# Aaron20127/human-3d-reconstruction

Hardware: AMD Instinct MI355X
Metric: images/sec whole-node, DLA-34+SMPL batch-64 512x512; top-k index bit-match (higher is better)
Workload: dtype bf16; 1 GPU; DLA-34+DCNv2 multi_pose + pose/shape heads -> sigmoid/NMS/top-100 decode -> SMPL 6890-vert LBS; 512x512, batch 64 per GPU (BASELINE configs[2]); batch_per_gpu=64, global_batch=64, K=100, smpl_people_per_image=100, parallelism=dp1 (image shards, one all-gather of dets), collective=none (one rank), steps_in_flight=3, hip_graph=False, dcn_margin=auto, images=64 distinct synthetic images (h3d_amd.synth.synth_image_batch, seed 317), weights=synthetic (h3d_amd.synth, seed 0, gain 1.25, offset_scale 0.5)

## Files before the change

human-3d-reconstruction_amd/_lib.py:

```python
import ctypes
import os

_HERE = os.path.dirname(os.path.abspath(__file__))
LIB_PATH = os.path.join(_HERE, "csrc", "libh3d_hip.so")

H3D_F32, H3D_BF16, H3D_F16, H3D_F16X3 = 0, 1, 2, 3
OP_STEM, OP_CONV, OP_DCN, OP_MAXPOOL, OP_UPADD, OP_COPY, OP_HEADS, OP_DCN_V1, OP_DCN_FUSED = 1, 2, 3, 4, 5, 6, 7, 8, 9
OP_CONV_STREAM, OP_DCN_FUSED_F16, OP_DCN_FUSED_STREAM, OP_STEM3, OP_UPDCN_F16 = 10, 11, 12, 13, 14
OP_IM2COL, OP_MAXPOOL3, OP_DEPTH2SPACE = 15, 16, 17
HEADS_MAX = 16
OUT_NHWC, OUT_NCHW_F32, OUT_NHWC_F32, OUT_NHWC_F16 = 0, 1, 2, 3
DCN_INPUT_NHWC, DCN_OUTPUT_NHWC, DCN_F32_MFMA = 1, 2, 4
ABI_VERSION = 4

DCN_AUX_BYTES = 256
DCN_FUSED_BIAS_WMAX, DCN_FUSED_BIAS_AMAX = 32, 34
OPF_DCN_MASK_FINAL, OPF_DCN_RAW_PACK, OPF_DCN_ACT_MAXIMA, TUNE_DCN_ABLATE_MASK = 0x800, 0x100000, 0x200000, 0x1f
OPF_DCN_FUSED_RAW_PACK, OPF_DCN_FUSED_SCALED_INPUT = 0x100000, 0x200000
TUNE_DCN_FUSED_X3_MARGIN2, TUNE_DCN_FUSED_X3_MARGIN6, TUNE_DCN_FUSED_X3_MARGIN4, TUNE_DCN_FUSED_X3_ABLATE_MASK = 0x2000, 0x4000, 0x8000, 0x1f
OPF_DCN_STREAM_NO_SLOTS, OPF_DCN_STREAM_WIDE_MARGIN, OPF_DCN_STREAM_SLOTS512, OPF_DCN_STREAM_F16_INPUT = 0x1000, 0x8000, 0x10000, 0x40000
OPF_DCN_STREAM_STATS, OPF_DCN_STREAM_VARIANT_MASK = 0x20000, 0x58600
TUNE_DCN_STREAM_FORCE_NARROW_WG, TUNE_DCN_STREAM_FORCE_WIDE_WG = 0x200, 0x400
TUNE_DCN_STREAM_F16_DCN5, TUNE_DCN_STREAM_F16_KEEP_DCN3, TUNE_DCN_STREAM_ABLATE_MASK = 0x4000, 0x2000, 0x1f
TUNE_DCN_STREAM_X3_MARGIN2, TUNE_DCN_STREAM_X3_MARGIN3, TUNE_DCN_STREAM_X3_MARGIN4, TUNE_DCN_STREAM_X3_ABLATE_MASK = 0x4000, 0x8000, 0x10000, 0x1f
TUNE_DCN_F16_ONE_WG_PER_CU, TUNE_DCN_F16_ABLATE_MASK = 0x100, 0xff
TUNE_CONV_STREAM_TILE_MASK, TUNE_CONV_STREAM_AUTO, TUNE_CONV_STREAM_ROUND4_RULE, TUNE_CONV_STREAM_ABLATE_MASK = 0xffff, 1, 0x10000000, 0x1f0000
TUNE_CONV_TILE, TUNE_CONV_HALO_TILE, TUNE_CONV_FORCE_GEMM, TUNE_CONV_GEMM_TILE_MASK = 0x1000, 0x2000, 0x4000, 0xf00
TUNE_CONV_X3_TILED, TUNE_CONV_X3_TILE_MASK, TUNE_CONV_X3_CK16, TUNE_CONV_X3_MT2 = 0x1000, 0x1fff, 0x2000, 0x4000
TUNE_UPADD_TAPS_GLOBAL, TUNE_UPADD_TAPS_LDS = 1, 2
TUNE_HEADS_SEPARATE_BIAS, TUNE_HEADS_ABLATE_MASK = 0x200, 0xff


def TUNE_DCN_STREAM_DCN5_XP(xp):
    return xp << 16


def TUNE_DCN_STREAM_DCN5_XP_OF(reserved):
    return (reserved >> 16) & 0xff


def TUNE_CONV_STREAM_TILE(variant, mt, waves):
    return variant << 12 | mt << 8 | waves


def TUNE_CONV_STREAM_ABLATE(bits):
    return bits << 16


def TUNE_CONV_STREAM_ABLATE_OF(reserved):
    return (reserved & TUNE_CONV_STREAM_ABLATE_MASK) >> 16


def TUNE_CONV_1X1_TILE(mt, th):
    return TUNE_CONV_TILE | mt << 4 | th >> 3


def TUNE_CONV_1X1_TILE_MT(reserved):
    return (reserved >> 4) & 15


def TUNE_CONV_1X1_TILE_TH(reserved):
    return (reserved & 15) * 8


def TUNE_CONV_GEMM_TILE(n):
    return n << 8


def TUNE_CONV_X3_TILE(mt, waves, th):
    return TUNE_CONV_X3_TILED | mt << 8 | waves << 4 | th >> 3

c_vp, c_i, c_fp = ctypes.c_void_p, ctypes.c_int, ctypes.c_void_p


class H3dOp(ctypes.Structure):
    _fields_ = [
        ("kind", ctypes.c_int32), ("dtype", ctypes.c_int32),
        ("in_", c_vp), ("in2", c_vp), ("w", c_vp), ("bias", c_vp), ("out", c_vp),
        ("B", ctypes.c_int32), ("H", ctypes.c_int32), ("W", ctypes.c_int32),
        ("Cin", ctypes.c_int32), ("in_cs", ctypes.c_int32), ("in2_cs", ctypes.c_int32),
        ("Ho", ctypes.c_int32), ("Wo", ctypes.c_int32),
        ("Cout", ctypes.c_int32), ("out_cs", ctypes.c_int32),
        ("ksize", ctypes.c_int32), ("stride", ctypes.c_int32), ("relu", ctypes.c_int32),
        ("out_mode", ctypes.c_int32), ("wrows", ctypes.c_int32), ("reserved", ctypes.c_int32),
        ("wexp", ctypes.c_int32), ("wexp2", ctypes.c_int32),
    ]


class _HeadEntry(ctypes.Structure):
    _fields_ = [("w2", c_vp), ("b2", c_vp), ("out", c_vp), ("C", ctypes.c_int32), ("wexp2", ctypes.c_int32)]


class H3dHeadsDesc(ctypes.Structure):
    _fields_ = [("nheads", ctypes.c_int32), ("wexp", ctypes.c_int32), ("head", _HeadEntry * HEADS_MAX)]


HEADS_LISTS_MAX = 4


class H3dHeadsList(ctypes.Structure):
    _fields_ = [("inds", c_vp), ("K", ctypes.c_int32), ("head_mask", ctypes.c_uint32)]


class H3dUpdcnDesc(ctypes.Structure):
    _fields_ = [("skip", c_vp), ("w_up", c_vp), ("w_off", c_vp), ("skip_cs", ctypes.c_int32), ("reserved", ctypes.c_int32)]


TRAIN_BRIGHTNESS, TRAIN_CONTRAST, TRAIN_SATURATION = 0, 1, 2
TRAIN_INPUT_NO_COLOR_AUG = 1


class H3dTrainImage(ctypes.Structure):
    _fields_ = [("minv", ctypes.c_double * 6), ("light", ctypes.c_double * 3), ("offset", ctypes.c_int64),
# ... 164 lines not shown
```

human-3d-reconstruction_amd/csrc/heads.hip:

```cpp
#include "common.h"
#include <string.h>
#include <type_traits>
#include <utility>

constexpr int HEADS_MAX = 16;
constexpr int HC_IN = 64;
constexpr int HC_SLAB = 64;
constexpr int HC_MT2 = 3;
constexpr int HEADS_LISTS_MAX = 4;
#ifndef HEADS_PF_WIDE
#define HEADS_PF_WIDE 0
#endif
#ifndef HEADS_PF
#define HEADS_PF 2
#endif

#ifndef HEADS_SPARSE_NW
#define HEADS_SPARSE_NW 8
#endif
static_assert(HEADS_SPARSE_NW == 4 || HEADS_SPARSE_NW == 8, "sparse heads: 24 wave-instructions per stage in whole numbers per wave, at most 512 threads");

struct HeadsArgs {
    const char *in;
    const char *w1;
    const float *b1;
    const char *w2[HEADS_MAX];
    const float *b2[HEADS_MAX];
    float *out[HEADS_MAX];
    int C[HEADS_MAX];
    int nheads, head_conv;
    int B, H, W, in_cs;
    int tiles_x, tiles_y;
    int dbg;
    int xcd;
    float s1;
    float s2[HEADS_MAX];
    unsigned long long *stamps;
    int nlists;
    const long long *l_inds[HEADS_LISTS_MAX];
    int l_K[HEADS_LISTS_MAX], l_wg0[HEADS_LISTS_MAX], l_nh[HEADS_LISTS_MAX];
    int l_head[HEADS_LISTS_MAX][HEADS_MAX];
};

template <typename T, int TH>
struct HeadsCfg {
    static constexpr int TW = 32;
    static constexpr int ES = sizeof(T);
    static constexpr int NT = TH / 8;
    static constexpr int NW = 8;
    static constexpr int IN_H = TH + 2, IN_W = TW + 2;
    static constexpr int SB = HC_IN * ES + 16;
    static constexpr int RB = IN_W * SB;
    static constexpr int RBW = HC_IN * ES;
    static constexpr int CPR = RBW / 16;
    static constexpr int SWZ_SHIFT = ES == 2 ? 1 : 0;
    static constexpr int TAPS = ES == 2 ? 3 : 1;
    static constexpr int TRS = 9 / TAPS;
    static constexpr int SLOT = TAPS * HC_SLAB * RBW;
    static constexpr int LDS_IN = IN_H * RB;
    static constexpr int LDS_W2 = 32 * HC_MT2 * RBW;
    static constexpr int LDS_BIAS = 1024 + 1024;
    static constexpr int LDS = LDS_IN + 2 * SLOT + LDS_W2 + 2 * LDS_BIAS;
    static constexpr int RPI = 1024 / RBW;
    static constexpr int VPR = HC_IN * ES / 16;
};

template <typename T>
struct HeadsSparseCfg {
    using D = HeadsCfg<T, 16>;
    static_assert(sizeof(T) == 2, "sparse heads: 2-byte plans");
    static constexpr int ES = D::ES, NT = 1, TW = D::TW;
    static constexpr int CW = 2, NW = HEADS_SPARSE_NW;
    static constexpr int NPOS = 32 * CW;
    static constexpr int SB = D::SB, RB = 3 * SB, PB = 3 * RB;
    static constexpr int RBW = D::RBW, CPR = D::CPR, SWZ_SHIFT = D::SWZ_SHIFT, TAPS = D::TAPS, TRS = D::TRS, SLOT = D::SLOT;
    static constexpr int LDS_IN = NPOS * PB;
    static constexpr int LDS_W2 = D::LDS_W2, LDS_BIAS = D::LDS_BIAS;
    static constexpr int LDS = LDS_IN + 2 * SLOT + LDS_W2 + 2 * LDS_BIAS;
    static constexpr int RPI = D::RPI, VPR = D::VPR;
    static_assert(LDS <= 160 * 1024, "LDS of a CU");
};

template <int OFF>
__device__ __forceinline__ void lds_read16_async(u32x4 &dst, uint32_t addr)
{
    static_assert(OFF >= 0 && OFF < 65536, "ds_read offset field");
    asm volatile("ds_read_b128 %0, %1 offset:%2" : "=v"(dst) : "v"(addr), "n"(OFF));
}
template <class F, int... I>
__device__ __forceinline__ void static_for_impl(F &&f, std::integer_sequence<int, I...>) { (f(std::integral_constant<int, I>{}), ...); }
template <int N, class F>
__device__ __forceinline__ void static_for(F &&f) { static_for_impl(f, std::make_integer_sequence<int, N>{}); }

__device__ __forceinline__ void heads_issue_bias(const float *b1, int hc, const float *b2, char *dst, int wv, int l)
{
    if (wv == 0) {
        const auto rs = __builtin_amdgcn_make_buffer_rsrc((void *)b1, 0, hc * 4, 0x00020000);
        __builtin_amdgcn_raw_ptr_buffer_load_lds(rs, (__attribute__((address_space(3))) void *)dst, 16, l * 16, 0, 0, 0);
    } else if (wv == 1) {
        const auto rs = __builtin_amdgcn_make_buffer_rsrc((void *)b2, 0, 96 * 4, 0x00020000);
        __builtin_amdgcn_raw_ptr_buffer_load_lds(rs, (__attribute__((address_space(3))) void *)(dst + 1024), 16, l * 16 < 512 ? l * 16 : 0x7ffffff0, 0, 0, 0);
    }
}

template <typename T, int TH, int NT, int M2, bool BIASC>
__device__ __forceinline__ void gemm2(f32x16 (&acc)[2][NT], f32x16 (&acc2)[M2][NT], const char *s_b1 ,
                                      const char *s_w2, int r, int h, int sw, float s1 = 1.f)
{
    using C = HeadsCfg<T, TH>;
    using E = ET<T>;
    constexpr int ES = sizeof(T);
    typedef short s16x2 __attribute__((ext_vector_type(2)));
#pragma unroll
    for (int m = 0; m < 2; ++m) {
#pragma unroll
        for (int sb = 0; sb < 2; ++sb) {
            typename E::frag fb[NT];
            float bias[8] = {0.f, 0.f, 0.f, 0.f, 0.f, 0.f, 0.f, 0.f};
            if constexpr (!BIASC) {
                const f32x4 b_lo = *reinterpret_cast<const f32x4 *>(s_b1 + (m * 32 + 16 * sb + 4 * h) * 4);
                const f32x4 b_hi = *reinterpret_cast<const f32x4 *>(s_b1 + (m * 32 + 16 * sb + 4 * h + 8) * 4);
#pragma unroll
                for (int j = 0; j < 4; ++j) { bias[j] = b_lo[j]; bias[4 + j] = b_hi[j]; }
// ... 363 lines not shown
                else if ((H3D_DBG(a) & 8) && wv < 4) {  }
                else if (BIASC && tr == 0) stage(std::true_type{}, slot, tr);
                else stage(std::false_type{}, slot, tr);
#ifdef H3D_ABLATE
                t_stage += __builtin_readcyclecounter() - ts0;
#endif
#ifdef H3D_ABLATE
                const unsigned long long tb0 = __builtin_readcyclecounter();
                __builtin_amdgcn_s_waitcnt(0x0f70);
                const unsigned long long tb1 = __builtin_readcyclecounter();
                t_dma += tb1 - tb0;
#endif
                if (!(H3D_DBG(a) & 2))
                __syncthreads();
#ifdef H3D_ABLATE
                t_bar += __builtin_readcyclecounter() - tb1;
#endif
            }
#ifdef H3D_ABLATE
            const unsigned long long tg0 = __builtin_readcyclecounter();
#endif
            if (!(SPARSE && idle))
            gemm2<T, TH, NT, M2H, BIASC>(acc, acc2, s_b + slab * HC_SLAB * 4, s_w2, r, h, sw, a.s1);
#ifdef H3D_ABLATE
            t_g2 += __builtin_readcyclecounter() - tg0;
#endif
            if (C::TRS == 1) __syncthreads();
        }
        const int C_head = a.C[head];
        float *out = a.out[head];
        const size_t cstride = (size_t)a.H * a.W;
        [[maybe_unused]] const float s2 = a.s2[head];
#pragma unroll
        for (int n = 0; n < NT; ++n) {
            const int oy = SPARSE ? sp_y : oy0 + wv * NT + n, ox = SPARSE ? sp_x : ox0 + r, ob = SPARSE ? sp_b : b;
            if (SPARSE ? sp_ok : oy < a.H && ox < a.W) {
                float *op = out + (((size_t)ob * C_head + 4 * h) * a.H + oy) * a.W + ox;
#pragma unroll
                for (int m2 = 0; m2 < M2H; ++m2) {
#pragma unroll
                    for (int g = 0; g < 4; ++g) {
                        const int c = m2 * 32 + 8 * g + 4 * h;
                        float *p = op + (size_t)(m2 * 32 + 8 * g) * cstride;
                        const f32x4 b2v = *reinterpret_cast<const f32x4 *>(s_b + 1024 + c * 4);
#pragma unroll
                        for (int i = 0; i < 4; ++i)
                            if (c + i < C_head) {
                                if constexpr (std::is_same_v<T, x3_t>) p[i * cstride] = fmaf(acc2[m2][n][4 * g + i], s2, b2v[i]);
                                else p[i * cstride] = acc2[m2][n][4 * g + i] + b2v[i];
                            }
                        __builtin_amdgcn_sched_barrier(0);
                    }
                }
            }
        }
        };
    for (int hi = 0; hi < nh; ++hi) {
        const int head = head_at(hi);
        if constexpr (!MIXED) {
            head_body(std::integral_constant<int, M2>{}, hi, head);
        } else {
            const int m2h = __builtin_amdgcn_readfirstlane((a.C[head] + 31) >> 5);
            if (m2h <= 1) head_body(std::integral_constant<int, 1>{}, hi, head);
            else if (M2 < 3 || m2h == 2) head_body(std::integral_constant<int, (M2 < 2 ? 1 : 2)>{}, hi, head);
            else head_body(std::integral_constant<int, M2>{}, hi, head);
        }
    }
#ifdef H3D_ABLATE
    if (a.stamps && blockIdx.x < 65536) {
        if (a.dbg & 64) {
            if (l == 0) a.stamps[blockIdx.x * H3D_NSTAMP + wv] = t_bar;
        } else if (tid == 0) {
            a.stamps[blockIdx.x * H3D_NSTAMP + 0] = t_start;
            a.stamps[blockIdx.x * H3D_NSTAMP + 1] = __builtin_readcyclecounter();
            a.stamps[blockIdx.x * H3D_NSTAMP + 2] = t_bar;
            a.stamps[blockIdx.x * H3D_NSTAMP + 3] = t_g2;
            a.stamps[blockIdx.x * H3D_NSTAMP + 4] = t_dma;
            a.stamps[blockIdx.x * H3D_NSTAMP + 5] = t_stage;
        }
    }
#endif
}

static_assert(HEADS_MAX == H3D_HEADS_MAX, "header/kernel mismatch");

static int heads_args(const h3d_op &op, HeadsArgs &a)
{
    if (!op.in || !op.w || !op.bias || !op.in2) H3D_FAIL(H3D_ERR_ARG, "heads: null pointer");
    const h3d_heads_desc *d = (const h3d_heads_desc *)op.in2;
    const int es = h3d_dtype_bytes(op.dtype);
    if (!es) H3D_FAIL(H3D_ERR_DTYPE, "heads: dtype %d", op.dtype);
    if (op.Cin != HC_IN || op.in_cs % (16 / es) || op.in_cs < HC_IN)
        H3D_FAIL(H3D_ERR_SHAPE, "heads: input must have %d channels (got %d, stride %d)", HC_IN, op.Cin, op.in_cs);
    if (op.Cout <= 0 || op.Cout % HC_SLAB || op.Cout > 256)
        H3D_FAIL(H3D_ERR_SHAPE, "heads: head_conv %d must be a multiple of %d, at most 256", op.Cout, HC_SLAB);
    if (d->nheads <= 0 || d->nheads > HEADS_MAX) H3D_FAIL(H3D_ERR_SHAPE, "heads: %d heads (max %d)", d->nheads, HEADS_MAX);
    a.in = (const char *)op.in; a.w1 = (const char *)op.w; a.b1 = op.bias;
    a.dbg = op.reserved & H3D_TUNE_HEADS_ABLATE_MASK;
    a.xcd = h3d_xcd_mode();
#ifdef H3D_ABLATE
    a.stamps = h3d_stamp_buffer();
#else
    a.stamps = nullptr;
#endif
    a.nlists = 0;
    memset(a.l_inds, 0, sizeof a.l_inds); memset(a.l_K, 0, sizeof a.l_K); memset(a.l_wg0, 0, sizeof a.l_wg0);
    memset(a.l_nh, 0, sizeof a.l_nh); memset(a.l_head, 0, sizeof a.l_head);
    a.nheads = d->nheads; a.head_conv = op.Cout; a.B = op.B; a.H = op.H; a.W = op.W; a.in_cs = op.in_cs;
    for (int i = 0; i < d->nheads; ++i) {
        if (!d->head[i].w2 || !d->head[i].b2 || !d->head[i].out) H3D_FAIL(H3D_ERR_ARG, "heads: head %d null pointer", i);
        if (d->head[i].C <= 0 || d->head[i].C > 32 * HC_MT2)
            H3D_FAIL(H3D_ERR_UNSUPPORTED, "heads: head %d has %d channels (max %d)", i, d->head[i].C, 32 * HC_MT2);
        a.w2[i] = (const char *)d->head[i].w2; a.b2[i] = d->head[i].b2; a.out[i] = d->head[i].out; a.C[i] = d->head[i].C;
        if (d->head[i].wexp2 < -60 || d->head[i].wexp2 > 60 || (d->head[i].wexp2 && op.dtype != H3D_F16X3))
            H3D_FAIL(H3D_ERR_ARG, "heads: head %d wexp2 %d (an H3D_F16X3 filter exponent)", i, d->head[i].wexp2);
        a.s2[i] = ldexpf(1.f, -d->head[i].wexp2);
    }
    if (d->wexp < -60 || d->wexp > 60 || (d->wexp && op.dtype != H3D_F16X3)) H3D_FAIL(H3D_ERR_ARG, "heads: wexp %d (an H3D_F16X3 filter exponent)", d->wexp);
    a.s1 = ldexpf(1.f, -d->wexp);
    return H3D_OK;
}

int h3d_launch_heads(const h3d_op &op, hipStream_t st)
{
    HeadsArgs a;
    if (const int rc = heads_args(op, a)) return rc;
    const h3d_heads_desc *d = (const h3d_heads_desc *)op.in2;
    const int es = h3d_dtype_bytes(op.dtype);
    int m2 = 1, m2min = HC_MT2;
    for (int i = 0; i < d->nheads; ++i) {
        m2 = max(m2, (d->head[i].C + 31) / 32);
        m2min = min(m2min, (d->head[i].C + 31) / 32);
    }
    const bool mixed = m2min != m2 && es == 2;
    const bool biasc = !(op.reserved & H3D_TUNE_HEADS_SEPARATE_BIAS);
    return h3d_by_dtype<bf16_t, f16_t, float, x3_t>(op.dtype, "heads: dtype %d", [&](auto t) {
        using T = typename decltype(t)::type;
        constexpr int TH = sizeof(T) == 2 ? 16 : 8;
        a.tiles_x = cdiv(op.W, 32); a.tiles_y = cdiv(op.H, TH);
        const dim3 grid(op.B * a.tiles_x * a.tiles_y), blk(512);
        return h3d_by_values([&](auto m2c, auto bc, auto mx) {
            const h3d_kname name{"heads_kernel", t, TH, m2c, bc, h3d_opt(mx)};
            if constexpr (mx && (m2c < 2 || !bc)) {
                if (name.dry()) return H3D_OK;
                H3D_FAIL(H3D_ERR_UNSUPPORTED, "heads: the separate-bias tuning override applies to launches of equal-width heads");
            } else {
                return h3d_launch(name, heads_kernel<T, TH, m2c, bc, mx>, grid, blk, 0, st, a);
            }
        }, h3d_vals<1, 2, 3>{}, m2, h3d_vals<false, true>{}, biasc, std::conditional_t<sizeof(T) == 2, h3d_vals<false, true>, h3d_vals<false>>{}, mixed);
    });
}

static_assert(HEADS_LISTS_MAX == H3D_HEADS_LISTS_MAX, "header/kernel mismatch");

extern "C" int h3d_heads_sparse_lists(const h3d_op *op, int nlists, const h3d_heads_list *lists, void *stream)
{
    if (!op || !lists) H3D_FAIL(H3D_ERR_ARG, "heads_sparse: null pointer");
    if (op->kind != H3D_OP_HEADS) H3D_FAIL(H3D_ERR_ARG, "heads_sparse: op kind %d is not H3D_OP_HEADS", op->kind);
    if (nlists <= 0 || nlists > HEADS_LISTS_MAX) H3D_FAIL(H3D_ERR_ARG, "heads_sparse: %d position lists (1..%d)", nlists, HEADS_LISTS_MAX);
    if (op->B <= 0 || op->H <= 0 || op->W <= 0) H3D_FAIL(H3D_ERR_SHAPE, "heads_sparse: B %d, H %d, W %d", op->B, op->H, op->W);
    for (int i = 0; i < nlists; ++i) {
        if (!lists[i].inds) H3D_FAIL(H3D_ERR_ARG, "heads_sparse: list %d null pointer", i);
        if (lists[i].K <= 0 || (long long)op->B * lists[i].K > (1 << 24))
            H3D_FAIL(H3D_ERR_SHAPE, "heads_sparse: list %d: B %d, K %d", i, op->B, lists[i].K);
    }
    if (op->dtype != H3D_BF16 && op->dtype != H3D_F16)
        H3D_FAIL(H3D_ERR_UNSUPPORTED, "heads_sparse: dtype %d (the 2-byte plans)", op->dtype);
    if (op->reserved) H3D_FAIL(H3D_ERR_UNSUPPORTED, "heads_sparse: tuning word %#x", (unsigned)op->reserved);
    HeadsArgs a;
    if (const int rc = heads_args(*op, a)) return rc;
    uint32_t seen = 0;
    for (int i = 0; i < nlists; ++i) {
        const uint32_t m = lists[i].head_mask;
        if (!m || (a.nheads < 32 && m >> a.nheads))
            H3D_FAIL(H3D_ERR_ARG, "heads_sparse: list %d head mask %#x (bits 0..%d of the op's %d heads, at least one)", i, (unsigned)m, a.nheads - 1, a.nheads);
        if (m & seen) H3D_FAIL(H3D_ERR_ARG, "heads_sparse: list %d head mask %#x names a head of an earlier list (%#x)", i, (unsigned)m, (unsigned)(m & seen));
        seen |= m;
    }
    int order[HEADS_LISTS_MAX];
    for (int i = 0; i < nlists; ++i) order[i] = i;
    for (int i = 1; i < nlists; ++i)
        for (int j = i; j > 0 && __builtin_popcount(lists[order[j]].head_mask) > __builtin_popcount(lists[order[j - 1]].head_mask); --j)
            std::swap(order[j], order[j - 1]);
    a.tiles_x = a.tiles_y = 1;
    return h3d_by_dtype<bf16_t, f16_t>(op->dtype, "heads_sparse: dtype %d", [&](auto t) {
        using T = typename decltype(t)::type;
        using C = HeadsSparseCfg<T>;
        int wgs = 0;
        a.nlists = nlists;
        for (int i = 0; i < nlists; ++i) {
            const h3d_heads_list &ls = lists[order[i]];
            a.l_inds[i] = (const long long *)ls.inds; a.l_K[i] = ls.K; a.l_wg0[i] = wgs; a.l_nh[i] = 0;
            for (int h = 0; h < a.nheads; ++h)
                if (ls.head_mask >> h & 1) a.l_head[i][a.l_nh[i]++] = h;
            wgs += cdiv(op->B * ls.K, C::NPOS);
        }
        const dim3 grid(wgs), blk(64 * C::NW);
        const h3d_kname name{"heads_kernel", t, 16, 3, true, h3d_opt(true), h3d_opt(true)};
        return h3d_launch(name, heads_kernel<T, 16, 3, true, true, true>, grid, blk, 0, (hipStream_t)stream, a);
    });
}

extern "C" int h3d_heads_sparse(const h3d_op *op, const int64_t *inds, int K, void *stream)
{
    if (!op || !inds) H3D_FAIL(H3D_ERR_ARG, "heads_sparse: null pointer");
    if (op->kind != H3D_OP_HEADS || !op->in2) H3D_FAIL(H3D_ERR_ARG, "heads_sparse: op kind %d is not H3D_OP_HEADS with a descriptor", op->kind);
    const int n = ((const h3d_heads_desc *)op->in2)->nheads;
    const h3d_heads_list all = {inds, K, n >= 32 ? ~0u : n > 0 ? (1u << n) - 1 : 1u};
    return h3d_heads_sparse_lists(op, 1, &all, stream);
}
```

include/h3d.h:

```cpp
#ifndef H3D_H
#define H3D_H

#include <stddef.h>
#include <stdint.h>

#ifdef __cplusplus
extern "C" {
#endif

#define H3D_OK 0
#define H3D_ERR_SHAPE (-1)
#define H3D_ERR_DTYPE (-2)
#define H3D_ERR_LAUNCH (-3)
#define H3D_ERR_UNSUPPORTED (-4)
#define H3D_ERR_ARG (-5)

#define H3D_F32 0
#define H3D_BF16 1
#define H3D_F16 2
#define H3D_F16X3 3

const char *h3d_last_error(void);
int h3d_abi_version(void);
#define H3D_ABI_VERSION 4
// ... 128 lines not shown
#define H3D_DCN_AUX_BYTES 256
#define H3D_DCN_FUSED_BIAS_WMAX 32
#define H3D_DCN_FUSED_BIAS_AMAX 34

enum {
    H3D_OPF_DCN_MASK_FINAL = 0x800,
    H3D_OPF_DCN_RAW_PACK = 0x100000,
    H3D_OPF_DCN_ACT_MAXIMA = 0x200000,
    H3D_TUNE_DCN_ABLATE_MASK = 0x1f
};

enum {
    H3D_OPF_DCN_FUSED_RAW_PACK = 0x100000,
    H3D_OPF_DCN_FUSED_SCALED_INPUT = 0x200000,
    H3D_TUNE_DCN_FUSED_X3_MARGIN2 = 0x2000,
    H3D_TUNE_DCN_FUSED_X3_MARGIN6 = 0x4000,
    H3D_TUNE_DCN_FUSED_X3_MARGIN4 = 0x8000,
    H3D_TUNE_DCN_FUSED_X3_ABLATE_MASK = 0x1f
};

enum {
    H3D_OPF_DCN_STREAM_NO_SLOTS = 0x1000,
    H3D_OPF_DCN_STREAM_WIDE_MARGIN = 0x8000,
    H3D_OPF_DCN_STREAM_SLOTS512 = 0x10000,
    H3D_OPF_DCN_STREAM_F16_INPUT = 0x40000,
    H3D_OPF_DCN_STREAM_STATS = 0x20000,
    H3D_OPF_DCN_STREAM_VARIANT_MASK = 0x58600,
    H3D_TUNE_DCN_STREAM_FORCE_NARROW_WG = 0x200,
    H3D_TUNE_DCN_STREAM_FORCE_WIDE_WG = 0x400,
    H3D_TUNE_DCN_STREAM_F16_DCN5 = 0x4000,
    H3D_TUNE_DCN_STREAM_F16_KEEP_DCN3 = 0x2000,
    H3D_TUNE_DCN_STREAM_ABLATE_MASK = 0x1f
};
#define H3D_TUNE_DCN_STREAM_DCN5_XP(xp) ((xp) << 16)
#define H3D_TUNE_DCN_STREAM_DCN5_XP_OF(reserved) (((reserved) >> 16) & 0xff)

enum {
    H3D_TUNE_DCN_STREAM_X3_MARGIN2 = 0x4000,
    H3D_TUNE_DCN_STREAM_X3_MARGIN3 = 0x8000,
    H3D_TUNE_DCN_STREAM_X3_MARGIN4 = 0x10000,
    H3D_TUNE_DCN_STREAM_X3_ABLATE_MASK = 0x1f
};

enum {
    H3D_TUNE_DCN_F16_ONE_WG_PER_CU = 0x100,
    H3D_TUNE_DCN_F16_ABLATE_MASK = 0xff
};

#define H3D_TUNE_CONV_STREAM_TILE(variant, mt, waves) ((variant) << 12 | (mt) << 8 | (waves))
#define H3D_TUNE_CONV_STREAM_ABLATE(bits) ((bits) << 16)
#define H3D_TUNE_CONV_STREAM_ABLATE_OF(reserved) (((reserved) & H3D_TUNE_CONV_STREAM_ABLATE_MASK) >> 16)
enum {
    H3D_TUNE_CONV_STREAM_TILE_MASK = 0xffff,
    H3D_TUNE_CONV_STREAM_AUTO = 1,
    H3D_TUNE_CONV_STREAM_ROUND4_RULE = 0x10000000,
    H3D_TUNE_CONV_STREAM_ABLATE_MASK = 0x1f0000
};

#define H3D_TUNE_CONV_1X1_TILE(mt, th) (H3D_TUNE_CONV_TILE | (mt) << 4 | (th) >> 3)
#define H3D_TUNE_CONV_1X1_TILE_MT(reserved) (((reserved) >> 4) & 15)
#define H3D_TUNE_CONV_1X1_TILE_TH(reserved) (((reserved) & 15) * 8)
#define H3D_TUNE_CONV_GEMM_TILE(n) ((n) << 8)
enum {
    H3D_TUNE_CONV_TILE = 0x1000,
    H3D_TUNE_CONV_HALO_TILE = 0x2000,
    H3D_TUNE_CONV_FORCE_GEMM = 0x4000,
    H3D_TUNE_CONV_GEMM_TILE_MASK = 0xf00
};
#define H3D_TUNE_CONV_X3_TILE(mt, waves, th) (H3D_TUNE_CONV_X3_TILED | (mt) << 8 | (waves) << 4 | (th) >> 3)
enum {
    H3D_TUNE_CONV_X3_TILED = 0x1000,
    H3D_TUNE_CONV_X3_TILE_MASK = 0x1fff,
    H3D_TUNE_CONV_X3_CK16 = 0x2000,
    H3D_TUNE_CONV_X3_MT2 = 0x4000
};

enum {
    H3D_TUNE_UPADD_TAPS_GLOBAL = 1,
    H3D_TUNE_UPADD_TAPS_LDS = 2
};

enum {
    H3D_TUNE_HEADS_SEPARATE_BIAS = 0x200,
    H3D_TUNE_HEADS_ABLATE_MASK = 0xff
};

int h3d_dcn_fused_ck(int Cin, int Cout);

int h3d_dcn_far_samples(const h3d_op *op, int32_t *per_tile, void *stream);

int h3d_run_ops(const h3d_op *ops, int n, void *stream);

int h3d_run_ops_timed(const h3d_op *ops, int n, void *stream, float *ms);
int h3d_op_kernel_name(const h3d_op *op, char *buf, int buflen);

int h3d_heads_sparse(const h3d_op *op, const int64_t *inds, int K, void *stream);

#define H3D_HEADS_LISTS_MAX 4
typedef struct h3d_heads_list {
    const int64_t *inds;
    int32_t K;
    uint32_t head_mask;
} h3d_heads_list;
int h3d_heads_sparse_lists(const h3d_op *op, int nlists, const h3d_heads_list *lists, void *stream);

int h3d_nchw_f32_to_nhwc(const float *src, void *dst, int dtype, int B, int C, int H, int W,
                         int dst_cs, void *stream);
int h3d_nhwc_to_nchw_f32(const void *src, int dtype, float *dst, int B, int C, int H, int W,
                         int src_cs, void *stream);

typedef struct h3d_heads_bwd_head {
    const float *w1, *b1, *w2;
    const float *grad_out;
    float *grad_w1, *grad_b1, *grad_w2, *grad_b2;
    int32_t C;
    int32_t reserved;
} h3d_heads_bwd_head;
int h3d_heads_backward_workspace_bytes(int B, int H, int W, int head_conv, int nheads, const int *C, size_t *bytes);
int h3d_heads_backward(const float *feat, int in_cs, int B, int H, int W, int head_conv, int nheads, const h3d_heads_bwd_head *heads,
                       float *grad_feat, void *workspace, size_t workspace_bytes, void *stream);

enum {
    H3D_CONV_BWD_RELU = 1
};
#define H3D_CONV_BWD_MFMA_CMAX 2048
int h3d_conv2d_backward_workspace_bytes(int B, int C, int H, int W, int Cout, int kh, int kw, int sh, int sw, int ph, int pw, int dh, int dw,
                                        int flags, size_t *bytes);
int h3d_conv2d_backward(const float *x, int x_cs, const float *weight, const float *y, int y_cs, const float *grad_y, int gy_cs,
                        float *grad_x, float *grad_res, float *grad_weight, float *grad_bias, int B, int C, int H, int W, int Cout,
                        int kh, int kw, int sh, int sw, int ph, int pw, int dh, int dw, int flags, void *workspace, size_t workspace_bytes,
                        void *stream);
int h3d_conv2d_backward_general(const float *x, int x_cs, const float *weight, const float *y, int y_cs, const float *grad_y, int gy_cs,
                                float *grad_x, float *grad_res, float *grad_weight, float *grad_bias, int B, int C, int H, int W, int Cout,
                                int kh, int kw, int sh, int sw, int ph, int pw, int dh, int dw, int flags, void *workspace,
                                size_t workspace_bytes, void *stream);


#define H3D_NMS_SIGMOID 1
#define H3D_NMS_SKIP 2
int h3d_nms_topk(const float *heat, int B, int C, int H, int W, int K, int flags,
                 float *scores, int64_t *inds, float *ys, float *xs, void *stream);
int h3d_nms_topk2(const float *heat_a, int Ca, float *scores_a, int64_t *inds_a, float *ys_a, float *xs_a,
                  const float *heat_b, int Cb, float *scores_b, int64_t *inds_b, float *ys_b, float *xs_b,
                  int B, int H, int W, int K, int flags, void *stream);

size_t h3d_nms_topk_large_workspace_bytes(int B, int C, int H, int W, int K);
int h3d_nms_topk_large(const float *heat, int B, int C, int H, int W, int K, int flags,
                       float *scores, int64_t *inds, float *ys, float *xs,
                       void *workspace, size_t workspace_bytes, void *stream);

int h3d_nms(const float *heat, int B, int C, int H, int W, float *out, void *stream);
int h3d_sigmoid_clamp(const float *in, float *out, size_t n, void *stream);

int h3d_topk_merge(const float *scores, const int64_t *inds, const float *ys, const float *xs,
                   int B, int C, int K, float *o_score, int64_t *o_ind, int32_t *o_cls,
                   float *o_y, float *o_x, void *stream);

int h3d_gather_feat(const float *feat, const int64_t *ind, int B, int C, int HW, int N,
                    int channels_last, float *out, void *stream);

int h3d_multi_pose_assemble(const float *c_score, const int64_t *c_ind, const int32_t *c_cls,
                            const float *c_y, const float *c_x,
                            const float *hp_score, const int64_t *hp_ind, const float *hp_y,
                            const float *hp_x,
                            const float *wh, const float *hps, const float *reg,
                            const float *hp_offset,
// ... 176 lines not shown
```

Baseline: 10570 images/s.

## Add register-resident sparse heads kernel with one workgroup per head and position group

Adds a new sparse heads kernel that loads each position's 3x3x64 input patch straight into registers with buffer loads, instead of staging patches in LDS. Work is split per head and per group of positions, with heads ordered by output tile count, and multi-tile outputs are parked in LDS between slabs. The aim is to cut LDS patch staging and to let each workgroup stream only its own head's weights. The cost is that each head's work group reloads the input patch, register pressure rises, and the launch is larger. It becomes the default whenever the input fits a 2 GiB buffer descriptor, with tuning flags to fall back to the old kernel or use 4 waves.

New measurement: 10720 images/s, median of 6. 1.01x the previous value.

```diff
diff --git a/human-3d-reconstruction_amd/_lib.py b/human-3d-reconstruction_amd/_lib.py
--- a/human-3d-reconstruction_amd/_lib.py
+++ b/human-3d-reconstruction_amd/_lib.py
@@ -29,6 +29,7 @@
 TUNE_CONV_X3_TILED, TUNE_CONV_X3_TILE_MASK, TUNE_CONV_X3_CK16, TUNE_CONV_X3_MT2 = 0x1000, 0x1fff, 0x2000, 0x4000
 TUNE_UPADD_TAPS_GLOBAL, TUNE_UPADD_TAPS_LDS = 1, 2
 TUNE_HEADS_SEPARATE_BIAS, TUNE_HEADS_ABLATE_MASK = 0x200, 0xff
+TUNE_HEADS_SPARSE_LDS_PATCH, TUNE_HEADS_SPARSE_WAVES4 = 0x400, 0x800
 
 
 def TUNE_DCN_STREAM_DCN5_XP(xp):
diff --git a/human-3d-reconstruction_amd/csrc/heads.hip b/human-3d-reconstruction_amd/csrc/heads.hip
--- a/human-3d-reconstruction_amd/csrc/heads.hip
+++ b/human-3d-reconstruction_amd/csrc/heads.hip
@@ -19,6 +19,9 @@
 #define HEADS_SPARSE_NW 8
 #endif
 static_assert(HEADS_SPARSE_NW == 4 || HEADS_SPARSE_NW == 8, "sparse heads: 24 wave-instructions per stage in whole numbers per wave, at most 512 threads");
+#ifndef HEADS_SPARSE_PF
+#define HEADS_SPARSE_PF 2
+#endif
 
 struct HeadsArgs {
     const char *in;
@@ -39,6 +42,7 @@
     int nlists;
     const long long *l_inds[HEADS_LISTS_MAX];
     int l_K[HEADS_LISTS_MAX], l_wg0[HEADS_LISTS_MAX], l_nh[HEADS_LISTS_MAX];
+    int l_ng[HEADS_LISTS_MAX];
     int l_head[HEADS_LISTS_MAX][HEADS_MAX];
 };
 
@@ -568,6 +572,199 @@
 #endif
 }
 
+template <typename T, int NW>
+struct HeadsSparseRegCfg {
+    using D = HeadsCfg<T, 16>;
+    static_assert(sizeof(T) == 2, "sparse heads: 2-byte plans");
+    static constexpr int ES = D::ES;
+    static constexpr int NPOS = 32 * NW;
+    static constexpr int RBW = D::RBW, CPR = D::CPR, SWZ_SHIFT = D::SWZ_SHIFT, TAPS = D::TAPS, TRS = D::TRS, SLOT = D::SLOT;
+    static_assert(TAPS == 3 && TRS == 3, "a stage is one tap row");
+    static constexpr int NFRAG = 9 * (HC_IN / 16);
+    static constexpr int LDS_W2 = D::LDS_W2, LDS_BIAS = D::LDS_BIAS;
+    static constexpr int LDS_PARK = NW * HC_MT2 * 16 * 256;
+    static constexpr int LDS = 2 * SLOT + LDS_W2 + LDS_BIAS + LDS_PARK;
+    static_assert(LDS <= 160 * 1024, "LDS of a CU");
+    static constexpr unsigned OUTSIDE = 0x80000000u;
+};
+constexpr size_t HEADS_SPARSE_REG_MAX_BYTES = (size_t)1 << 31;
+
+template <typename T, int NW>
+__global__ __launch_bounds__(64 * NW, NW == 8 ? 2 : 1) void heads_sparse_kernel(HeadsArgs a)
+{
+    using C = HeadsSparseRegCfg<T, NW>;
+    using E = ET<T>;
+    constexpr int ES = C::ES;
+    __shared__ __attribute__((aligned(16))) char smem[C::LDS];
+    char *s_ring = smem;
+    char *s_w2 = s_ring + 2 * C::SLOT;
+    char *s_bias = s_w2 + C::LDS_W2;
+    char *s_park = s_bias + C::LDS_BIAS;
+
+    const int tid = threadIdx.x;
+    const int wv = tid >> 6, l = tid & 63, r = l & 31, h = l >> 5;
+    const int wvs = __builtin_amdgcn_readfirstlane(wv);
+    const int bid = blockIdx.x;
+    int li = 0;
+#pragma unroll
+    for (int i = 1; i < HEADS_LISTS_MAX; ++i)
+        if (i < a.nlists && bid >= a.l_wg0[i]) li = i;
+    const int lb = bid - a.l_wg0[li], ng = a.l_ng[li];
+    const int hi = lb / ng, grp = lb - hi * ng;
+    const int head = a.l_head[li][hi];
+    const int sp_K = a.l_K[li];
+    const long long *sp_inds = a.l_inds[li];
+    const int slabs = a.head_conv / HC_SLAB;
+    const int nstages = slabs * C::TRS;
+    const int sw = (r >> C::SWZ_SHIFT) & (C::CPR - 1);
+
+    const int w1_bytes = a.nheads * a.head_conv * 9 * HC_IN * ES;
+    auto issue_w1 = [&](int s) {
+        const int slab = s / C::TRS, tr = s - slab * C::TRS;
+        heads_dma_w1<T, 16, NW>(a.w1, w1_bytes, s_ring + (s & 1) * C::SLOT, wvs, l, (((head * slabs + slab) * HC_SLAB * 9 + tr * C::TAPS) * HC_IN) * ES);
+    };
+    issue_w1(0);
+    heads_issue_bias(a.b1 + head * a.head_conv, a.head_conv, a.b2[head], s_bias, wvs, l);
+
+    int sp_b = 0, sp_y = 0, sp_x = 0;
+    bool sp_ok = false;
+    const int p = grp * C::NPOS + wv * 32 + r;
+    if (p < a.B * sp_K) {
+        const long long ind = sp_inds[p];
+        if (ind >= 0 && ind < (long long)a.H * a.W) { sp_ok = true; sp_b = p / sp_K; sp_y = (int)ind / a.W; sp_x = (int)ind - sp_y * a.W; }
+    }
+    u32x4 bf[C::NFRAG];
+    {
+        const size_t in_bytes = (((size_t)a.B * a.H * a.W - 1) * a.in_cs + HC_IN) * ES;
+        const auto rs = __builtin_amdgcn_make_buffer_rsrc((void *)a.in, 0, (int)in_bytes, 0x00020000);
+#pragma unroll
+        for (int tap = 0; tap < 9; ++tap) {
+            const int gy = sp_y - 1 + tap / 3, gx = sp_x - 1 + tap % 3;
+            const bool inside = sp_ok && gy >= 0 && gy < a.H && gx >= 0 && gx < a.W;
+            const unsigned off = inside ? (unsigned)((((sp_b * a.H + gy) * a.W + gx) * a.in_cs + 8 * h) * ES) : C::OUTSIDE;
+#pragma unroll
+            for (int kk = 0; kk < HC_IN / 16; ++kk)
+                bf[tap * (HC_IN / 16) + kk] = __builtin_bit_cast(u32x4, __builtin_amdgcn_raw_buffer_load_b128(rs, off + kk * 16 * ES, 0, 0));
+        }
+    }
+    __syncthreads();
+
+    auto body = [&](auto m2_tag) {
+        constexpr int M2H = decltype(m2_tag)::value;
+        constexpr bool PARK = M2H > 1;
+        char *park = s_park + (wv * HC_MT2 * 16 * 64 + l * 4) * 4;
+        auto park_tile = [&](int m2, const f32x16 &t) {
+#pragma unroll
+            for (int q = 0; q < 4; ++q) *reinterpret_cast<f32x4 *>(park + (m2 * 4 + q) * 1024) = f32x4{t[4 * q], t[4 * q + 1], t[4 * q + 2], t[4 * q + 3]};
+        };
+        auto parked_tile = [&](int m2, f32x16 &t) {
+#pragma unroll
+            for (int q = 0; q < 4; ++q) {
+                const f32x4 v = *reinterpret_cast<const f32x4 *>(park + (m2 * 4 + q) * 1024);
+#pragma unroll
+                for (int i = 0; i < 4; ++i) t[4 * q + i] = v[i];
+            }
+        };
+        f32x16 acc[2][1], acc2[1][1];
+#pragma unroll
+        for (int m = 0; m < 2; ++m)
+#pragma unroll
+            for (int i = 0; i < 16; ++i) acc[m][0][i] = 0.f;
+#pragma unroll
+        for (int i = 0; i < 16; ++i) acc2[0][0][i] = 0.f;
+        int s = 0;
+        for (int slab = 0; slab < slabs; ++slab) {
+            auto stage = [&](auto tr_tag) {
+                constexpr int TR = decltype(tr_tag)::value;
+                if (s + 1 < nstages) issue_w1(s + 1);
+                if (TR == 1) heads_dma_w2<T, 16, NW>(a.w2[head], a.head_conv, s_w2, wvs, l, slab * HC_SLAB * ES);
+                const char *slot = s_ring + (s & 1) * C::SLOT;
+                auto load_bias = [&](f32x16 &dst, int m) {
+#pragma unroll
+                    for (int g = 0; g < 4; ++g) {
+                        const f32x4 bv = *reinterpret_cast<const f32x4 *>(s_bias + (slab * HC_SLAB + m * 32 + 8 * g + 4 * h) * 4);
+#pragma unroll
+                        for (int i = 0; i < 4; ++i) dst[4 * g + i] = bv[i];
+                    }
+                };
+                constexpr int NSTEP = C::TAPS * (HC_IN / 16);
+                const uint32_t ring = (uint32_t)(uintptr_t)(__attribute__((address_space(3))) const char *)slot + r * C::RBW;
+                uint32_t fa_base[HC_IN / 16];
+#pragma unroll
+                for (int kk = 0; kk < HC_IN / 16; ++kk) fa_base[kk] = ring + (((2 * kk + h) ^ sw) << 4);
+                constexpr int PF = HEADS_SPARSE_PF, NBUF = PF + 1;
+                static_assert(PF * 2 <= 15, "lgkmcnt field");
+                u32x4 fa[NBUF][2];
+                auto fetch = [&](auto step_tag) {
+                    constexpr int STEP = decltype(step_tag)::value, BUF = STEP % NBUF;
+                    constexpr int tp = STEP / (HC_IN / 16), kk = STEP - tp * (HC_IN / 16);
+                    lds_read16_async<(tp * HC_SLAB) * C::RBW>(fa[BUF][0], fa_base[kk]);
+                    lds_read16_async<(tp * HC_SLAB + 32) * C::RBW>(fa[BUF][1], fa_base[kk]);
+                };
+                static_for<PF>([&](auto step_tag) { fetch(step_tag); });
+                static_for<NSTEP>([&](auto step_tag) {
+                    constexpr int STEP = decltype(step_tag)::value, BUF = STEP % NBUF;
+                    if constexpr (STEP + PF < NSTEP) fetch(std::integral_constant<int, STEP + PF>{});
+                    constexpr int NEWER = (STEP + PF < NSTEP ? PF : NSTEP - 1 - STEP) * 2;
+                    __builtin_amdgcn_s_waitcnt(0xc07f | (NEWER << 8));
+                    __builtin_amdgcn_sched_barrier(0);
+#pragma unroll
+                    for (int m = 0; m < 2; ++m) {
+                        if (TR == 0 && STEP == 0) { load_bias(acc[m][0], m); }
+                        typename E::frag a_, b_;
+                        a_.v = fa[BUF][m]; b_.v = bf[TR * NSTEP + STEP];
+                        E::mma(acc[m][0], a_, b_);
+                    }
+                    __builtin_amdgcn_sched_barrier(0);
+                });
+                __syncthreads();
+                ++s;
+            };
+            stage(std::integral_constant<int, 0>{});
+            stage(std::integral_constant<int, 1>{});
+            stage(std::integral_constant<int, 2>{});
+            if constexpr (!PARK) {
+                gemm2<T, 16, 1, 1, true>(acc, acc2, s_bias + slab * HC_SLAB * 4, s_w2, r, h, sw, a.s1);
+            } else {
+#pragma unroll
+                for (int m2 = 0; m2 < M2H; ++m2) {
+                    if (slab == 0) {
+#pragma unroll
+                        for (int i = 0; i < 16; ++i) acc2[0][0][i] = 0.f;
+                    } else {
+                        parked_tile(m2, acc2[0][0]);
+                    }
+                    gemm2<T, 16, 1, 1, true>(acc, acc2, s_bias + slab * HC_SLAB * 4, s_w2 + m2 * 32 * C::RBW, r, h, sw, a.s1);
+                    park_tile(m2, acc2[0][0]);
+                }
+            }
+        }
+        if (sp_ok) {
+            const int C_head = a.C[head];
+            const size_t cstride = (size_t)a.H * a.W;
+            float *op = a.out[head] + (((size_t)sp_b * C_head + 4 * h) * a.H + sp_y) * a.W + sp_x;
+#pragma unroll
+            for (int m2 = 0; m2 < M2H; ++m2) {
+                if (PARK) parked_tile(m2, acc2[0][0]);
+#pragma unroll
+                for (int g = 0; g < 4; ++g) {
+                    const int c = m2 * 32 + 8 * g + 4 * h;
+                    float *q = op + (size_t)(m2 * 32 + 8 * g) * cstride;
+                    const f32x4 b2v = *reinterpret_cast<const f32x4 *>(s_bias + 1024 + c * 4);
+#pragma unroll
+                    for (int i = 0; i < 4; ++i)
+                        if (c + i < C_head) q[i * cstride] = acc2[0][0][4 * g + i] + b2v[i];
+                    __builtin_amdgcn_sched_barrier(0);
+                }
+            }
+        }
+    };
+    const int m2h = __builtin_amdgcn_readfirstlane((a.C[head] + 31) >> 5);
+    if (m2h <= 1) body(std::integral_constant<int, 1>{});
+    else if (m2h == 2) body(std::integral_constant<int, 2>{});
+    else body(std::integral_constant<int, 3>{});
+}
+
 static_assert(HEADS_MAX == H3D_HEADS_MAX, "header/kernel mismatch");
 
 static int heads_args(const h3d_op &op, HeadsArgs &a)
@@ -591,7 +788,7 @@
 #endif
     a.nlists = 0;
     memset(a.l_inds, 0, sizeof a.l_inds); memset(a.l_K, 0, sizeof a.l_K); memset(a.l_wg0, 0, sizeof a.l_wg0);
-    memset(a.l_nh, 0, sizeof a.l_nh); memset(a.l_head, 0, sizeof a.l_head);
+    memset(a.l_nh, 0, sizeof a.l_nh); memset(a.l_head, 0, sizeof a.l_head); memset(a.l_ng, 0, sizeof a.l_ng);
     a.nheads = d->nheads; a.head_conv = op.Cout; a.B = op.B; a.H = op.H; a.W = op.W; a.in_cs = op.in_cs;
     for (int i = 0; i < d->nheads; ++i) {
         if (!d->head[i].w2 || !d->head[i].b2 || !d->head[i].out) H3D_FAIL(H3D_ERR_ARG, "heads: head %d null pointer", i);
@@ -652,7 +849,8 @@
     }
     if (op->dtype != H3D_BF16 && op->dtype != H3D_F16)
         H3D_FAIL(H3D_ERR_UNSUPPORTED, "heads_sparse: dtype %d (the 2-byte plans)", op->dtype);
-    if (op->reserved) H3D_FAIL(H3D_ERR_UNSUPPORTED, "heads_sparse: tuning word %#x", (unsigned)op->reserved);
+    if (op->reserved & ~(H3D_TUNE_HEADS_SPARSE_LDS_PATCH | H3D_TUNE_HEADS_SPARSE_WAVES4))
+        H3D_FAIL(H3D_ERR_UNSUPPORTED, "heads_sparse: tuning word %#x", (unsigned)op->reserved);
     HeadsArgs a;
     if (const int rc = heads_args(*op, a)) return rc;
     uint32_t seen = 0;
@@ -669,11 +867,34 @@
         for (int j = i; j > 0 && __builtin_popcount(lists[order[j]].head_mask) > __builtin_popcount(lists[order[j - 1]].head_mask); --j)
             std::swap(order[j], order[j - 1]);
     a.tiles_x = a.tiles_y = 1;
+    a.nlists = nlists;
+    const size_t in_bytes = (((size_t)op->B * op->H * op->W - 1) * op->in_cs + HC_IN) * h3d_dtype_bytes(op->dtype);
+    if (!(op->reserved & H3D_TUNE_HEADS_SPARSE_LDS_PATCH) && in_bytes < HEADS_SPARSE_REG_MAX_BYTES) {
+        const bool waves8 = !(op->reserved & H3D_TUNE_HEADS_SPARSE_WAVES4);
+        const int npos = 32 * (waves8 ? 8 : 4);
+        int wgs = 0;
+        for (int i = 0; i < nlists; ++i) {
+            const h3d_heads_list &ls = lists[order[i]];
+            a.l_inds[i] = (const long long *)ls.inds; a.l_K[i] = ls.K; a.l_wg0[i] = wgs; a.l_nh[i] = 0;
+            for (int tiles = HC_MT2; tiles >= 1; --tiles)
+                for (int h = 0; h < a.nheads; ++h)
+                    if ((ls.head_mask >> h & 1) && (a.C[h] + 31) / 32 == tiles) a.l_head[i][a.l_nh[i]++] = h;
+            a.l_ng[i] = cdiv(op->B * ls.K, npos);
+            wgs += a.l_nh[i] * a.l_ng[i];
+        }
+        return h3d_by_dtype<bf16_t, f16_t>(op->dtype, "heads_sparse: dtype %d", [&](auto t) {
+            using T = typename decltype(t)::type;
+            return h3d_by_values([&](auto nw) {
+                constexpr int NW = decltype(nw)::value;
+                const h3d_kname name{"heads_sparse_kernel", t, NW};
+                return h3d_launch(name, heads_sparse_kernel<T, NW>, dim3(wgs), dim3(64 * NW), 0, (hipStream_t)stream, a);
+            }, h3d_vals<4, 8>{}, waves8 ? 8 : 4);
+        });
+    }
     return h3d_by_dtype<bf16_t, f16_t>(op->dtype, "heads_sparse: dtype %d", [&](auto t) {
         using T = typename decltype(t)::type;
         using C = HeadsSparseCfg<T>;
         int wgs = 0;
-        a.nlists = nlists;
         for (int i = 0; i < nlists; ++i) {
             const h3d_heads_list &ls = lists[order[i]];
             a.l_inds[i] = (const long long *)ls.inds; a.l_K[i] = ls.K; a.l_wg0[i] = wgs; a.l_nh[i] = 0;
diff --git a/include/h3d.h b/include/h3d.h
--- a/include/h3d.h
+++ b/include/h3d.h
@@ -234,6 +234,8 @@
 
 enum {
     H3D_TUNE_HEADS_SEPARATE_BIAS = 0x200,
+    H3D_TUNE_HEADS_SPARSE_LDS_PATCH = 0x400,
+    H3D_TUNE_HEADS_SPARSE_WAVES4 = 0x800,
     H3D_TUNE_HEADS_ABLATE_MASK = 0xff
 };
 
```
